# Grice-Lab/HmmUFOtu

Measured on AMD Instinct MI355X. Metric: reads placed/sec (whole node), gg_97_otus GTR+dGamma 250bp; HBM GB/s %peak, higher is better.
Workload: dtype f64; 1 GPU; gg_97_otus-scale synthetic DB (198643 nodes x 7682 CS columns, K=1400), GTR+dGamma(4), SE 250 bp amplicon reads, batch 8192 reads/step/GPU, 6 batches in flight, seeds in the reference's std::sort order (k_seed_refsort); seed_order=reference, message_window_cols=7682, parallelism=read-sharded x1

## Files before the change

hmmufotu_amd/csrc/hu_engine.hip:

```cpp
#include <algorithm>
#include <cmath>
#include <cstdio>
#include <cstring>
#include <limits>
#include <map>
#include <atomic>
#include <thread>
#include <memory>
#include <mutex>
#include <chrono>
#include <fstream>
#include <sstream>
#include <new>
#include <stdexcept>
#include <fcntl.h>
#include <unistd.h>
#include "hu_common.h"
#include "hu_kern_sep.h"
#include "hu_kern_align.h"
#include "hu_kern_tree.h"
#include "hu_kern_blk.h"
#include "hu_kern_refsort.h"
#include "hu_kern_rank.h"
#include "hu_kern_anneal.h"
// ... 1667 lines not shown
	bool fixedRoot = false;
	bool placesGiven = false;
	bool pair16 = false;
	int scanWidth = 0;
	int pairsKind = 0;
	int seedCap = HU_MAX_SEEDS;
	hipStream_t stream = nullptr;
	hipEvent_t ev[2 * HU_T_COUNT];
	bool evSet[HU_T_COUNT] = {false};
	float ms[HU_T_COUNT];
	double wall[4] = {0, 0, 0, 0};
	DBuf<char> dBases, dTraces, dRows;
	DBuf<HuReadDesc> dDescs;
	DBuf<double> dScratch;
	DBuf<uint8_t> dDec;
	DBuf<HuVitOut> dVit;
	DBuf<HuAlnDev> dAlns;
	DBuf<int8_t> dCodes;
	DBuf<int32_t> dStart, dEnd, dSeedCnt, dSeedId, dGiven, dPermCnt;
	DBuf<uint16_t> dPerm;
	DBuf<uint32_t> dRp, dPairs, dSeedDN, dParDN, dBmin, dRSpan, dTileSpan;
	DBuf<int32_t> dTileQ, dSlotRead, dReadSlot;
	DBuf<uint32_t> dRq, dTileW;
	DBuf<unsigned long long> dRefScratch;
	DBuf<int32_t> dHv, dZeroPar; DBuf<unsigned long long> dPairsC; int refHvCount = 0; double refHvHeight = NAN;
	DBuf<int32_t> dBail, dNanCnt, dNanId; DBuf<uint32_t> dNanDN;
	int nRefBail = 0;
	DBuf<uint32_t> dRefPiv; DBuf<unsigned long long> dRefL0; bool refFused = false;
	int refHostAll = 0;
	DBuf<int32_t> dIns, dTileIns, dRetry;
	DBuf<uint32_t> dSortK, dSortV;
	DBuf<uint32_t> dCsCnt;
	DBuf<HuEstOut> dEst;
	DBuf<HuCand> dCands;
	DBuf<HuPlaceOut> dPlaceOut;
	DBuf<int32_t> dCandCnt, dCandOff, dMeta;
	DBuf<uint8_t> dFiltSlot;
	DBuf<HuPlaceRec> dPlaces;
	DBuf<hu_place_rec> dBest;
	size_t nc = 0;
	int maxGapSites = 0, maxBaseSites = 0;
	bool hostCands = false;
	DBuf<double> dRootLL;
	PinnedVec<double> hRootLL;
	std::vector<HuReadDesc> hDescs;
	std::vector<char> hBases;
	PinnedVec<HuVitOut> hVit;
	int64_t cellsTotal = 0, cornerTotal = 0;
	int rMain = 0;
	int maxAll = 1, maxMain = 1;
	std::vector<int32_t> wideReads;
	std::vector<uint32_t> hWideOrd, hWideCand; DBuf<uint32_t> dWideOrd, dWideCand;
	PinnedVec<int32_t> hCandOffAll;
	DBuf<double> dRedoScr; DBuf<HuReadDesc> dRedoDesc; DBuf<HuVitOut> dRedoVit;
	PinnedVec<HuAlnDev> hAlns;
	DBuf<int32_t> dAnRow, dAnThr, dAnTileQ; DBuf<int2> dAnReg; DBuf<uint32_t> dAnMasks; DBuf<unsigned long long> dAnHits;
	PinnedVec<int32_t> hStart, hEnd, hSeedCnt, hSeedId;
	PinnedVec<uint32_t> hSeedDN;
	PinnedVec<HuCand> hCands;
	std::vector<int64_t> candOffs;
	std::vector<HostPlace> places;
	PinnedVec<hu_place_rec> best;
	PinnedVec<int32_t> hMeta, hBail;
	PinnedVec<char> hRows;
	DBuf<uint32_t> dSumBits; DBuf<unsigned char> dSumCls; DBuf<int4> dSumOut; PinnedVec<int4> hSumOut; bool sumReady = false;
	std::vector<char> tsvBuf; std::vector<size_t> tsvOff, tsvLen; size_t tsvSize = 0;
// ... 955 lines not shown
	const int kth = tmp[W];
	static const int bounds[] = {512, 768, 1024, 1536, 2048, 3072};
	int bound = 0;
	for(int x : bounds) if(kth <= x) { bound = x; break; }
	if(!bound || bound >= b->maxAll) return;
	b->rMain = bound; b->maxMain = 1;
	for(int r = 0; r < b->n; ++r) { if(R[r] > bound) b->wideReads.push_back(r); else b->maxMain = std::max(b->maxMain, R[r]); }
	if(b->knob.trace) fprintf(stderr, "[hu] width split: %zu of %d reads beyond %d columns (widest %d) take a launch of their own\n", b->wideReads.size(), b->n, bound, b->maxAll);
}
static HuDbDev width_pass_dev(const hu_batch* b, int pass, const uint32_t* wideList) {
	HuDbDev dev = b->db->dev;
	if(b->rMain) { dev.rLo = pass ? b->rMain : -1; dev.rHi = pass ? 0x7fffffff : b->rMain; dev.wideList = pass ? wideList : nullptr; }
	return dev;
}

extern "C" int hu_estimate_batch(hu_batch* b, const hu_opts* o) try {
	if(!b || !o) return HU_ERR_ARG;
	if(b->state < ST_SEEDED) { hu_set_error("hu_estimate_batch: no seeds"); return HU_ERR_STATE; }
	HIPCHK(hipSetDevice(b->db->device));
	const size_t n = (size_t) b->n;
	int rc;
	if((rc = b->dEst.ensure(n * HU_MAX_SEEDS)) != HU_OK) return rc;
	(void) hipGetLastError();
	if(n) {
		Timer t(b, HU_T_ESTIMATE);
		plan_width_split(b);
		const bool stream = b->knob.streaming_sep != 0;
		if(b->rMain) {
			b->hWideOrd.clear();
			for(int r : b->wideReads) for(int sd = 0; sd < HU_MAX_SEEDS; ++sd) b->hWideOrd.push_back((uint32_t) r * HU_MAX_SEEDS + sd);
			if((rc = b->dWideOrd.ensure(b->hWideOrd.size())) != HU_OK) return rc;
			HIPCHK(hipMemcpyAsync(b->dWideOrd.p, b->hWideOrd.data(), b->hWideOrd.size() * 4, hipMemcpyHostToDevice, b->stream));
		}
		for(int pass = 0; pass < (b->rMain ? 2 : 1); ++pass) {
			const int maxR = pass ? b->maxAll : b->maxMain;
			const HuDbDev dev = width_pass_dev(b, pass, b->dWideOrd.p);
			#define EST_ARGS dev, b->db->mdl, b->dCodes.p, b->dStart.p, b->dEnd.p, b->dParDN.p, b->dSeedCnt.p, b->dSeedId.p, b->dSeedDN.p, o->weighted, b->dEst.p
			const unsigned eg = pass ? (unsigned) b->hWideOrd.size() : (unsigned) b->n * HU_MAX_SEEDS;
			const uint32_t* order = nullptr;
			if(pass) order = b->dWideOrd.p;
			else if(!b->knob.est_unsorted) {
				if((rc = b->dSortK.ensure((size_t) eg * 2)) != HU_OK || (rc = b->dSortV.ensure((size_t) eg * 2)) != HU_OK) return rc;
				k_seed_sortkeys<<<(eg + 255) / 256, 256, 0, b->stream>>>(b->n, b->dSeedCnt.p, b->dSeedId.p, b->dSortK.p, b->dSortV.p);
				if((rc = order_by_key(b, b->dSortK.p, b->dSortV.p, (size_t) eg, (uint32_t) b->db->dev.nNodes, b->dSortV.p + eg, false)) != HU_OK) return rc;
				order = b->dSortV.p + eg;
			}
			const int spt = (maxR + 255) / 256;
			const int xm = b->knob.xcd_map;
			const unsigned egl = pass ? eg : order ? std::min<unsigned>(eg, (unsigned) b->n * (unsigned) b->seedCap) : eg;
			const int var = b->knob.est_var;
			auto said = [&](const char* k) { if(b->knob.trace) fprintf(stderr, "[hu] estimate: max region %d, %s\n", maxR, k); };
			if(stream || spt > 12) { said("k_estimate"); k_estimate<<<eg, 64, 0, b->stream>>>(EST_ARGS); }
			else if(var == 2) {
				if(spt <= 2) { said("k_estimate_blk<2,256>"); k_estimate_blk<2, 256><<<eg, 256, 0, b->stream>>>(EST_ARGS); }
				else if(spt <= 4) { said("k_estimate_blk<4,256>"); k_estimate_blk<4, 256><<<eg, 256, 0, b->stream>>>(EST_ARGS); }
				else if(spt <= 6) { said("k_estimate_blk<6,256>"); k_estimate_blk<6, 256><<<eg, 256, 0, b->stream>>>(EST_ARGS); }
				else if(spt <= 8) { said("k_estimate_blk<8,256>"); k_estimate_blk<8, 256><<<eg, 256, 0, b->stream>>>(EST_ARGS); }
				else { said("k_estimate_blk<12,256>"); k_estimate_blk<12, 256><<<eg, 256, 0, b->stream>>>(EST_ARGS); }
			}
			else if(var == 98 && spt > 4 && spt <= 6) {
				said("k_estimate_prod<6,4,4,true>");
				DBuf<long long> ddb;
				if((rc = ddb.ensure((size_t) egl * 4)) != HU_OK) return rc;
				HIPCHK(hipMemsetAsync(ddb.p, 0, (size_t) egl * 4 * sizeof(long long), b->stream));
				k_estimate_prod<6, 4, 4, true><<<egl, 256, 0, b->stream>>>(EST_ARGS, order, xm, ddb.p);
				std::vector<long long> hd((size_t) egl * 4);
				HIPCHK(hipMemcpyAsync(hd.data(), ddb.p, hd.size() * sizeof(long long), hipMemcpyDeviceToHost, b->stream));
				HIPCHK(hu_wait(b->stream));
				double acc[4] = {0}; size_t ran = 0;
				for(size_t c = 0; c < (size_t) egl; ++c) if(hd[c * 4 + 3]) { ++ran; for(int i = 0; i < 4; ++i) acc[i] += (double) hd[c * 4 + i]; }
				if(ran) fprintf(stderr, "[est dbg] per slot (s_memtime ticks, %zu slots): prologue %.0f load %.0f rest %.0f total %.0f\n", ran, acc[0] / ran, acc[1] / ran, acc[2] / ran, acc[3] / ran);
			}
			else if(var == 1 && spt <= 6) { said("k_estimate_prod<12,2>"); k_estimate_prod<12, 2><<<egl, 128, 0, b->stream>>>(EST_ARGS, order, xm); }
			else if(var == 3 && spt <= 6) { said("k_estimate_prod<6,4,1>"); k_estimate_prod<6, 4, 1><<<egl, 256, 0, b->stream>>>(EST_ARGS, order, xm); }
			else if(spt <= 2) { said("k_estimate_prod<2,4>"); k_estimate_prod<2, 4><<<egl, 256, 0, b->stream>>>(EST_ARGS, order, xm); }
			else if(spt <= 4) { said("k_estimate_prod<4,4>"); k_estimate_prod<4, 4><<<egl, 256, 0, b->stream>>>(EST_ARGS, order, xm); }
			else if(spt <= 6) { said("k_estimate_prod<6,4,4>"); k_estimate_prod<6, 4, 4><<<egl, 256, (size_t)(b->knob.est_lds_pad > 0 && b->knob.est_lds_pad <= 60 ? b->knob.est_lds_pad : 0) * 1024, b->stream>>>(EST_ARGS, order, xm); }
			else if(spt <= 8) { said("k_estimate_prod<8,4>"); k_estimate_prod<8, 4><<<egl, 256, 0, b->stream>>>(EST_ARGS, order, xm); }
			else if(var == 4) { said("k_estimate_prod<12,4>"); k_estimate_prod<12, 4><<<egl, 256, 0, b->stream>>>(EST_ARGS, order, xm); }
			else { said("k_estimate_prod<6,8,2>"); k_estimate_prod<6, 8, 2><<<egl, 512, 0, b->stream>>>(EST_ARGS, order, xm); }
			#undef EST_ARGS
		}
	}
	HIPCHK(hipGetLastError());
	if(n) {
		if((rc = b->dPermCnt.ensure(n * 2)) != HU_OK) return rc;
		k_site_count<<<b->n, 64, 0, b->stream>>>(b->db->dev, b->n, b->dCodes.p, b->dStart.p, b->dEnd.p, b->dPermCnt.p);
		HIPCHK(hipGetLastError());
	}
	b->state = ST_ESTIMATED;
	return HU_OK;
} catch(...) { return hu_catch_all("hu_estimate_batch"); }


static int sync_host_cands(hu_batch* b) {
	if(b->hostCands) return HU_OK;
	const size_t n = (size_t) b->n;
	std::vector<int32_t> off(n + 1, 0);
	b->places.resize(b->nc);
	HIPCHK(hipSetDevice(b->db->device));
	if(n) HIPCHK(hipMemcpyAsync(off.data(), b->dCandOff.p, (n + 1) * 4, hipMemcpyDeviceToHost, b->stream));
	if(b->nc) HIPCHK(hipMemcpyAsync(b->places.data(), b->dPlaces.p, b->nc * sizeof(HuPlaceRec), hipMemcpyDeviceToHost, b->stream));
	HIPCHK(hu_wait(b->stream));
	b->candOffs.assign(off.begin(), off.end());
	b->hostCands = true;
	return HU_OK;
}
static int scan_cands(hu_batch* b, bool withPerm) {
	int rc;
	if((rc = b->dCandOff.ensure((size_t) b->n + 1)) != HU_OK || (rc = b->dMeta.ensure(4)) != HU_OK) return rc;
	k_cand_scan<<<1, 1024, 0, b->stream>>>(b->n, b->dCandCnt.p, b->dCandOff.p, withPerm ? b->dPermCnt.p : nullptr, b->dStart.p, b->dEnd.p, b->dMeta.p, b->rMain);
	HIPCHK(hipGetLastError());
	b->hMeta.assign(4, 0);
	int32_t* meta = b->hMeta.data();
// ... 708 lines not shown
		HIPCHK(hu_wait(b->stream));
	}
	for(size_t r = 0; r < n; ++r) {
		if(n_seeds) n_seeds[r] = cnt[r];
		for(int s = 0; s < HU_MAX_SEEDS && s < stride; ++s) {
			const bool ok = s < cnt[r];
			const size_t k = r * HU_MAX_SEEDS + s, w = r * (size_t) stride + s;
			if(ids) ids[w] = ok ? id[k] : -1;
			if(d) d[w] = ok ? (int32_t)(dn[k] >> 16) : 0;
			if(N) N[w] = ok ? (int32_t)(dn[k] & 0xffffu) : 0;
		}
	}
	return HU_OK;
} catch(...) { return hu_catch_all("hu_batch_get_seeds_strided"); }
extern "C" int hu_batch_get_estimates_strided(hu_batch* b, double* ratio, double* wnr, double* loglik, int stride) try {
	if(!b || stride < 1) return HU_ERR_ARG;
	if(b->state < ST_ESTIMATED) { hu_set_error("no estimates yet"); return HU_ERR_STATE; }
	HIPCHK(hipSetDevice(b->db->device));
	const size_t n = (size_t) b->n;
	std::vector<HuEstOut> e(n * HU_MAX_SEEDS); std::vector<int32_t> cnt(n);
	if(n) {
		HIPCHK(hipMemcpyAsync(e.data(), b->dEst.p, e.size() * sizeof(HuEstOut), hipMemcpyDeviceToHost, b->stream));
		HIPCHK(hipMemcpyAsync(cnt.data(), b->dSeedCnt.p, n * 4, hipMemcpyDeviceToHost, b->stream));
		HIPCHK(hu_wait(b->stream));
	}
	for(size_t r = 0; r < n; ++r) for(int s = 0; s < HU_MAX_SEEDS && s < stride; ++s) {
		const size_t k = r * HU_MAX_SEEDS + s, w = r * (size_t) stride + s; const bool ok = s < cnt[r];
		if(ratio) ratio[w] = ok ? e[k].ratio : NAN;
		if(wnr) wnr[w] = ok ? e[k].wnr : NAN;
		if(loglik) loglik[w] = ok ? e[k].loglik : NAN;
	}
	return HU_OK;
} catch(...) { return hu_catch_all("hu_batch_get_estimates_strided"); }
extern "C" int hu_batch_get_candidates(hu_batch* b, int64_t* offs, int32_t* c_node, double* ratio, double* wnr, double* est_loglik, int32_t* iters) try {
	if(!b) return HU_ERR_ARG;
	if(b->state < ST_FILTERED) { hu_set_error("no candidates yet"); return HU_ERR_STATE; }
	{ const int rc = sync_host_cands(b); if(rc != HU_OK) return rc; }
	if(offs) memcpy(offs, b->candOffs.data(), b->candOffs.size() * 8);
	for(size_t c = 0; c < b->places.size(); ++c) {
		const HostPlace& p = b->places[c];
		if(c_node) c_node[c] = p.cNode; if(ratio) ratio[c] = p.ratio; if(wnr) wnr[c] = p.wnr;
		if(est_loglik) est_loglik[c] = p.estLoglik; if(iters) iters[c] = p.iters;
	}
	return HU_OK;
} catch(...) { return hu_catch_all("hu_batch_get_candidates"); }
static hu_place_rec to_rec(const HostPlace& p, int32_t nCand) {
	hu_place_rec r;
	r.c_node = p.cNode; r.p_node = p.pNode; r.a_node = p.aNode; r.n_cand = nCand;
	r.wuv = p.wuv; r.ratio = p.ratio; r.wnr = p.wnr; r.loglik = p.loglik; r.height = p.height;
	r.q_place = p.qPlace; r.q_taxon = p.qTaxon; r.anno_dist = p.annoDist(); r.est_loglik = p.estLoglik; r.root_loglik = p.rootLoglik;
	return r;
}
extern "C" int hu_batch_get_candidate_places(hu_batch* b, hu_place_rec* recs) try {
	if(!b || !recs) return HU_ERR_ARG;
	if(b->state < ST_FINISHED) { hu_set_error("batch is not finished"); return HU_ERR_STATE; }
	{ const int rc = sync_host_cands(b); if(rc != HU_OK) return rc; }
	for(size_t r = 0; r + 1 < b->candOffs.size(); ++r)
		for(int64_t c = b->candOffs[r]; c < b->candOffs[r + 1]; ++c) recs[c] = to_rec(b->places[c], (int32_t)(b->candOffs[r + 1] - b->candOffs[r]));
	return HU_OK;
} catch(...) { return hu_catch_all("hu_batch_get_candidate_places"); }
extern "C" int hu_batch_get_placements(hu_batch* b, hu_place_rec* best) try {
	if(!b || !best) return HU_ERR_ARG;
	if(b->state < ST_FINISHED) { hu_set_error("batch is not finished"); return HU_ERR_STATE; }
	memcpy(best, b->best.data(), b->best.size() * sizeof(hu_place_rec));
	return HU_OK;
} catch(...) { return hu_catch_all("hu_batch_get_placements"); }
// ... 407 lines not shown
```

hmmufotu_amd/csrc/hu_kern_blk.h:

```cpp
#pragma once
#include "hu_kern_sep.h"

#define HU_BLK_THREADS 256

__device__ inline void lds_wave_sync() { asm volatile("s_waitcnt lgkmcnt(0)" ::: "memory"); }
__device__ inline void lds_barrier() { asm volatile("s_waitcnt lgkmcnt(0)\n\ts_barrier" ::: "memory"); }

template<int NW = 4>
__device__ inline double block_sum(double v, double* red, int& phase) {
	v = wave_sum_uniform(v);
	double* r = red + (phase & 1) * NW;
	if((threadIdx.x & 63) == 0) r[threadIdx.x >> 6] = v;
	lds_barrier();
	double s = r[0];
#pragma unroll
	for(int w = 1; w < NW; ++w) s += r[w];
	phase ^= 1;
	return s;
}
template<int NW = 4>
__device__ inline long long block_sum_ll(long long v, long long* red, int& phase) {
	for(int m = 32; m > 0; m >>= 1) v += __shfl_xor(v, m);
	long long* r = red + (phase & 1) * NW;
	if((threadIdx.x & 63) == 0) r[threadIdx.x >> 6] = v;
// ... 97 lines not shown
	if(tid == 0) { HuEstOut o; o.ratio = ratio; o.wnr = wnr; o.loglik = ll; out[(size_t) read * HU_MAX_SEEDS + s] = o; }
}

template<int CTRL>
__device__ inline double dpp_mul_full(double v) {
	const int lo = __builtin_amdgcn_mov_dpp(__double2loint(v), CTRL, 0xf, 0xf, true);
	const int hi = __builtin_amdgcn_mov_dpp(__double2hiint(v), CTRL, 0xf, 0xf, true);
	return v * __hiloint2double(hi, lo);
}
__device__ inline double wave_prod(double v) {
	v = dpp_mul_full<0xB1>(v);
	v = dpp_mul_full<0x4E>(v);
	v = dpp_mul_full<0x141>(v);
	v = dpp_mul_full<0x140>(v);
	v *= __shfl_xor(v, 16);
	v *= __shfl_xor(v, 32);
	return v;
}
__device__ inline int wave_sum_i32(int v) {
	for(int m = 32; m > 0; m >>= 1) v += __shfl_xor(v, m);
	return v;
}

__device__ inline uint32_t hu_xcd_pos(uint32_t b, uint32_t nb, int xmap) {
	if(!xmap) return b;
	const uint32_t per = nb >> 3;
	return b < per * 8 ? (b & 7u) * per + (b >> 3) : b;
}

__host__ __device__ constexpr int hu_est_waves(int spt, int occ) {
	const int w = spt <= 2 ? 8 : spt <= 4 ? 5 : spt <= 6 ? 4 : spt <= 8 ? 3 : 2;
	return occ > w ? occ : w;
}
template<int SPT, int NW, int OCC = 1, bool DBG = false>
__global__ __launch_bounds__(64 * NW, hu_est_waves(SPT, OCC)) void k_estimate_prod(HuDbDev db, HuModelDev mdl, const int8_t* __restrict__ codes,
		const int32_t* __restrict__ rstart, const int32_t* __restrict__ rend, const uint32_t* __restrict__ parDN,
		const int32_t* __restrict__ seedCnt, const int32_t* __restrict__ seedId, const uint32_t* __restrict__ seedDN,
		int weighted, HuEstOut* __restrict__ out, const uint32_t* __restrict__ order, int xmap = 0, long long* __restrict__ dbg = nullptr) {
	constexpr int THREADS = 64 * NW;
	long long tk[4] = {0, 0, 0, 0}, t0 = 0, tl = 0;
	auto stamp = [&](int i) { if(DBG) { const long long t = (long long) __builtin_amdgcn_s_memtime(); tk[i] += t - tl; tl = t; } };
	if(DBG) { t0 = tl = (long long) __builtin_amdgcn_s_memtime(); }
	__shared__ double redd[2 * NW];
	__shared__ int redi[2 * NW];
	__shared__ __attribute__((aligned(16))) double Qtab[24];
	__shared__ __attribute__((aligned(16))) double pro[12];
	__shared__ __attribute__((aligned(16))) double mtab[36];
	const uint32_t slot = order ? order[hu_xcd_pos(blockIdx.x, gridDim.x, xmap)] : blockIdx.x;
	const int read = slot / HU_MAX_SEEDS, s = slot % HU_MAX_SEEDS, tid = threadIdx.x, lane = tid & 63;
	const int wave = __builtin_amdgcn_readfirstlane(tid >> 6);
	const bool builder = wave == (int)(blockIdx.x % NW);
	if(s >= seedCnt[read] || hu_skip_width(db, rend[read] - rstart[read] + 1)) return;
	const int un = seedId[(size_t) read * HU_MAX_SEEDS + s];
	double ratio = 0;
	if(builder) {
		static_assert(offsetof(HuModelDev, U) == offsetof(HuModelDev, pi) + 64 && offsetof(HuModelDev, U1) == offsetof(HuModelDev, pi) + 192, "pi, logpi, U, U1 in a row");
		const double* __restrict__ mp = reinterpret_cast<const double*>(reinterpret_cast<const char*>(&mdl) + offsetof(HuModelDev, pi));
		const int l36 = lane < 36 ? lane : 0;
		const double mc = mp[l36 < 4 ? l36 : l36 + 4];
		const uint32_t dn = seedDN[(size_t) read * HU_MAX_SEEDS + s];
		const uint32_t pv = parDN[(size_t) read * HU_MAX_SEEDS + s];
		const double cDist = (double)(dn >> 16) / (double)(dn & 0xffffu);
		const double pDist = (double)(pv >> 16) / (double)(pv & 0xffffu);
		ratio = cDist / (cDist + pDist);
		if(isnan(ratio)) ratio = 0.5;
		ratio = __hiloint2double(__builtin_amdgcn_readfirstlane(__double2hiint(ratio)), __builtin_amdgcn_readfirstlane(__double2loint(ratio)));
		const double w0 = db.blen[un];
		const double wur = w0 * ratio, wvr = w0 - wur;
		const int l6 = lane < 6 ? lane : 0, m3 = l6 % 3;
		const double e = exp((m3 == 0 ? mdl.lam[1] : m3 == 1 ? mdl.lam[2] : mdl.lam[3]) * (l6 < 3 ? wur : wvr));
		if(lane < 6) pro[lane] = e;
		if(weighted) {
			double piw[4];
			{ double mx = max4d(mdl.logpi), sm; for(int i = 0; i < 4; ++i) piw[i] = exp(mdl.logpi[i] - mx); sm = (piw[0] + piw[2]) + (piw[1] + piw[3]); for(int i = 0; i < 4; ++i) piw[i] /= sm; }
			if(lane < 4) pro[8 + lane] = sel4(piw, lane);
		}
		if(lane < 36) mtab[lane] = mc;
	}
	const int start = rstart[read], end = rend[read], n = end - start + 1;
	const int8_t* __restrict__ cd = codes + (size_t) read * db.csLen + start;
	const int64_t sOff = (int64_t) un * db.winLen + (start - db.winStart);
	const int piMax = argmax4d(mdl.logpi);
	double z[SPT][4]; unsigned long long bop = 0; int ksum = 0;
	double Eu[3], Ev[3];
	double aU[SPT][4], aV[SPT][4];
	const double* __restrict__ Ub = db.up + sOff * 4; const double* __restrict__ Vb = db.down + sOff * 4;
	const int32_t* __restrict__ upKb = db.upK + sOff; const int32_t* __restrict__ downKb = db.downK + sOff;
	auto inr = [&](int t) { return tid < n - THREADS * t; };
	stamp(0);
	{
		int kU[SPT], kV[SPT];
#pragma unroll
		for(int t = 0; t < SPT; ++t) {
			const int jj = inr(t) ? tid + THREADS * t : 0;
			kU[t] = upKb[(size_t) jj]; kV[t] = downKb[(size_t) jj];
		}
		__builtin_amdgcn_sched_barrier(0);
#pragma unroll
		for(int t = 0; t < SPT; ++t) {
			const int jj = inr(t) ? tid + THREADS * t : 0;
			load4(Ub + (size_t) jj * 4, aU[t]); load4(Vb + (size_t) jj * 4, aV[t]);
			const int b = cd[jj];
			bop |= (unsigned long long)(b >= 0 ? b : 4) << (3 * t);
		}
		__builtin_amdgcn_sched_barrier(0);
		lds_barrier();
		{
			const double e = pro[lane < 6 ? lane : 0];
			const int lo = __double2loint(e), hi = __double2hiint(e);
#pragma unroll
			for(int k = 0; k < 3; ++k) {
				Eu[k] = __hiloint2double(__builtin_amdgcn_readlane(hi, k), __builtin_amdgcn_readlane(lo, k));
				Ev[k] = __hiloint2double(__builtin_amdgcn_readlane(hi, 3 + k), __builtin_amdgcn_readlane(lo, 3 + k));
			}
		}
#pragma unroll
		for(int t = 0; t < SPT; ++t) {
			asm volatile("" : "+v"(kU[t]), "+v"(kV[t]));
			ksum += inr(t) ? kU[t] + kV[t] : 0;
		}
	}
	if(DBG) { double x = 0; for(int t = 0; t < SPT; ++t) x += aU[t][0] + aV[t][0]; if(x == 1.2345e-300 || bop == ~0ull) tk[2] = 1; }
	stamp(1);
	{
#pragma unroll
		for(int t = 0; t < SPT; ++t) {
			const double su1 = Eu[0] * aU[t][1], su2 = Eu[1] * aU[t][2], su3 = Eu[2] * aU[t][3];
			const double sv1 = Ev[0] * aV[t][1], sv2 = Ev[1] * aV[t][2], sv3 = Ev[2] * aV[t][3];
#pragma unroll
			for(int i = 0; i < 4; ++i) {
				const double cu = fmax(fma(mdl.U[i*4+3], su3, fma(mdl.U[i*4+2], su2, fma(mdl.U[i*4+1], su1, aU[t][0]))), 0.0);
				const double cv = fmax(fma(mdl.U[i*4+3], sv3, fma(mdl.U[i*4+2], sv2, fma(mdl.U[i*4+1], sv1, aV[t][0]))), 0.0);
				z[t][i] = cu * cv;
			}
		}
	}
	double wnr = 0;
	if(!weighted) {
		int nd = 0;
#pragma unroll
		for(int t = 0; t < SPT; ++t) {
			const int bi = (int)((bop >> (3 * t)) & 7u);
			const int b1 = argmax4_tied_lin(z[t]), b2 = bi < 4 ? bi : piMax;
			nd += __popcll(__ballot(inr(t) && b1 != b2));
		}
		if(lane == 0) redi[wave] = nd;
		lds_barrier();
		if(builder) {
			int tot = redi[0];
#pragma unroll
			for(int w = 1; w < NW; ++w) tot += redi[w];
			wnr = (double) tot / (double) n;
		}
	}
	else {
		const double piwGap = pro[8 + piMax];
		double dsum = 0, nsum = 0;
#pragma unroll
		for(int t = 0; t < SPT; ++t) {
			if(!inr(t)) continue;
			const int bi = (int)((bop >> (3 * t)) & 7u);
			const int b1 = argmax4_tied_lin(z[t]), b2 = bi < 4 ? bi : piMax;
			const double w1 = sel4(z[t], b1) / ((z[t][0] + z[t][2]) + (z[t][1] + z[t][3]));
			const double w2 = bi < 4 ? 1.0 : piwGap;
			if(b1 != b2) dsum += w1 * w2;
			nsum += w1 * w2;
		}
		dsum = wave_sum(dsum); nsum = wave_sum(nsum);
		if(lane == 0) { redd[wave] = dsum; redd[NW + wave] = nsum; }
		lds_barrier();
		if(builder) {
			double a = redd[0], c = redd[NW];
#pragma unroll
			for(int w = 1; w < NW; ++w) { a += redd[w]; c += redd[NW + w]; }
			wnr = a / c;
		}
	}
	double* Q = Qtab;
	if(builder) {
		if(lane < 3) Q[1 + lane] = exp((lane == 0 ? mdl.lam[1] : lane == 1 ? mdl.lam[2] : mdl.lam[3]) * wnr);
		lds_wave_sync();
		if(lane < 20) {
			const int b = lane >> 2, i = lane & 3;
			const double* mU = mtab + 4 + i * 4, * mU1 = mtab + 20 + (b & 3);
			const double pii = mtab[i];
			double c;
			if(wnr == 0) c = b < 4 ? (i == b ? 1.0 : 0.0) : pii;
			else {
				double a0, a1, a2, a3;
				if(b < 4) { a0 = mU1[0]; a1 = mU1[4]; a2 = mU1[8]; a3 = mU1[12]; }
				else {
					a0 = (mdl.U1[0] * mdl.pi[0] + mdl.U1[1] * mdl.pi[1]) + (mdl.U1[2] * mdl.pi[2] + mdl.U1[3] * mdl.pi[3]);
					a1 = (mdl.U1[4] * mdl.pi[0] + mdl.U1[5] * mdl.pi[1]) + (mdl.U1[6] * mdl.pi[2] + mdl.U1[7] * mdl.pi[3]);
					a2 = (mdl.U1[8] * mdl.pi[0] + mdl.U1[9] * mdl.pi[1]) + (mdl.U1[10] * mdl.pi[2] + mdl.U1[11] * mdl.pi[3]);
					a3 = (mdl.U1[12] * mdl.pi[0] + mdl.U1[13] * mdl.pi[1]) + (mdl.U1[14] * mdl.pi[2] + mdl.U1[15] * mdl.pi[3]);
				}
				const double Ui1 = mU[1], Ui2 = mU[2], Ui3 = mU[3];
				c = fmax(fma(Ui3, Q[3] * a3, fma(Ui2, Q[2] * a2, fma(Ui1, Q[1] * a1, a0))), 0.0);
			}
			Q[4 + b * 4 + i] = pii * c;
		}
	}
	lds_barrier();
	double mant = 1.0; int esum = ksum;
#pragma unroll
	for(int t = 0; t < SPT; ++t) {
		const double* q = Q + 4 + ((bop >> (3 * t)) & 7u) * 4;
		double x = fmax(fma(q[3], z[t][3], fma(q[2], z[t][2], fma(q[1], z[t][1], q[0] * z[t][0]))), 0.0);
		if(!inr(t)) x = 1.0;
		mant *= __builtin_amdgcn_frexp_mant(x);
		esum += x == 0.0 ? 0 : __builtin_amdgcn_frexp_exp(x);
	}
	esum += __builtin_amdgcn_frexp_exp(mant); mant = __builtin_amdgcn_frexp_mant(mant);
	mant = wave_prod(mant);
	esum = wave_sum_i32(esum);
	if(lane == 0) { redd[wave] = mant; redi[NW + wave] = esum; }
	lds_barrier();
	if(builder && lane == 0) {
		double m = redd[0]; long long e = redi[NW];
#pragma unroll
		for(int w = 1; w < NW; ++w) { m *= redd[w]; e += redi[NW + w]; }
		HuEstOut o; o.ratio = ratio; o.wnr = wnr; o.loglik = log(m) + (double) e * HU_LN2;
		out[(size_t) read * HU_MAX_SEEDS + s] = o;
	}
	if(DBG) {
		stamp(2);
		if(builder && lane == 0) { tk[3] = tl - t0; for(int i = 0; i < 4; ++i) dbg[(size_t) blockIdx.x * 4 + i] = tk[i]; }
	}
}

#define HU_RHO_SKIP 1e60
#define HU_TP 18
#define HU_EXP_MEPS 0.99999000004999983333
#define HU_EXP_PEPS 1.00001000005000016667

__device__ inline double fast_div(double a, double b) {
	double y = __builtin_amdgcn_rcp(b);
	y = fma(fma(-b, y, 1.0), y, y);
	y = fma(fma(-b, y, 1.0), y, y);
	const double q = a * y;
	return fma(fma(-b, q, a), y, q);
}

__device__ __attribute__((noinline)) double hu_exp_call(double x) { return exp(x); }
__device__ __attribute__((noinline)) double hu_log_call(double x) { return log(x); }

template<int SPT, int NW, int EMV, int RED>
__device__ inline double em_branch_blk(const double (&rho)[SPT], int nvalidWave, double q0, double maxL,
		double* red, double* redc, int& phase, int& emIters, long long* st = nullptr) {
	long long tl = st ? (long long) __builtin_amdgcn_s_memtime() : 0;
	auto stamp = [&](int i) { if(st) { const long long t = (long long) __builtin_amdgcn_s_memtime(); st[i] += t - tl; tl = t; } };
	const int lane = threadIdx.x & 63, wave = threadIdx.x >> 6;
	double p0 = 1 - q0, p = p0, q = q0, rc = 0;
	const int em0 = emIters;
	if(lane == 0) redc[(phase & 1) * NW + wave] = (double) nvalidWave;
	for(int it = 0; it < HU_MAX_ITER && p >= 0 && p <= 1; ++it) {
// ... 330 lines not shown
```

hmmufotu_amd/engine.py:

```python
from __future__ import annotations

import ctypes as C
import os
import subprocess

import numpy as np

_HERE = os.path.dirname(os.path.abspath(__file__))
LIB_PATH = os.environ.get("HU_LIB") or os.path.join(_HERE, "libhmmufotu_amd.so")
_LIB = None

HU_MAX_SEEDS = 64
T_NAMES = ["viterbi", "align_build", "seed_pdist", "seed_topk", "estimate", "place", "_6", "_7"]
MODE = {"global": 0, "local": 1, "ngcl": 2, "cgnl": 3}


class EngineError(RuntimeError):
    pass


class ProfileDesc(C.Structure):
    _fields_ = [("K", C.c_int32), ("L", C.c_int32), ("EM", C.POINTER(C.c_double)), ("EI", C.POINTER(C.c_double)),
                ("T", C.POINTER(C.c_double)), ("p2cs", C.POINTER(C.c_int32))]

# ... 2320 lines not shown
        _chk(load_library().hu_anneal_batch(self.h, _p(rows, C.c_int32), C.c_int(n), txt, C.c_double(max_dist), _p(hn, C.c_int64), _p(hl, C.c_int64)))
        return hn, hl

    def pdist(self, read: int):
        d = np.zeros(self.db.n_nodes, np.int32); N = np.zeros(self.db.n_nodes, np.int32)
        _chk(load_library().hu_batch_get_pdist(self.h, C.c_int(read), _p(d, C.c_int32), _p(N, C.c_int32)))
        return d, N

    def seeds(self):
        n = self.n
        cnt = np.zeros(n, np.int32); ids = np.zeros((n, HU_MAX_SEEDS), np.int32); d = np.zeros_like(ids); N = np.zeros_like(ids)
        _chk(load_library().hu_batch_get_seeds(self.h, _p(cnt, C.c_int32), _p(ids, C.c_int32), _p(d, C.c_int32), _p(N, C.c_int32)))
        return cnt, ids, d, N

    def seeds_strided(self, stride: int, guard: int = 0):
        n = self.n
        cnt = np.zeros(n, np.int32)
        bufs = [np.full(n * stride + guard, -777, np.int32) for _ in range(3)]
        _chk(load_library().hu_batch_get_seeds_strided(self.h, _p(cnt, C.c_int32), *[_p(b, C.c_int32) for b in bufs], C.c_int(stride)))
        return (cnt,) + tuple(bufs)

    def estimates_strided(self, stride: int, guard: int = 0):
        n = self.n
        bufs = [np.full(n * stride + guard, -777.0) for _ in range(3)]
        _chk(load_library().hu_batch_get_estimates_strided(self.h, *[_p(b, C.c_double) for b in bufs], C.c_int(stride)))
        return tuple(bufs)

    def estimates(self):
        n = self.n
        r = np.zeros((n, HU_MAX_SEEDS)); w = np.zeros_like(r); ll = np.zeros_like(r)
        _chk(load_library().hu_batch_get_estimates(self.h, _p(r, C.c_double), _p(w, C.c_double), _p(ll, C.c_double)))
        return r, w, ll

    def candidates(self):
        offs = np.zeros(self.n + 1, np.int64)
        _chk(load_library().hu_batch_get_candidates(self.h, _p(offs, C.c_int64), None, None, None, None, None))
        m = int(offs[-1])
        c = np.zeros(m, np.int32); r = np.zeros(m); w = np.zeros(m); e = np.zeros(m); it = np.zeros(m, np.int32)
        _chk(load_library().hu_batch_get_candidates(self.h, _p(offs, C.c_int64), _p(c, C.c_int32), _p(r, C.c_double), _p(w, C.c_double),
                                                    _p(e, C.c_double), _p(it, C.c_int32)))
        return dict(offs=offs, c_node=c, ratio=r, wnr=w, est_loglik=e, iters=it)

    def placements(self):
        out = np.zeros(self.n, PLACE_DTYPE)
        _chk(load_library().hu_batch_get_placements(self.h, out.ctypes.data_as(C.c_void_p)))
        return out

    def candidate_places(self):
        offs = np.zeros(self.n + 1, np.int64)
        _chk(load_library().hu_batch_get_candidates(self.h, _p(offs, C.c_int64), None, None, None, None, None))
        out = np.zeros(int(offs[-1]), PLACE_DTYPE)
        _chk(load_library().hu_batch_get_candidate_places(self.h, out.ctypes.data_as(C.c_void_p)))
        return offs, out

    def set_candidates(self, offs, recs, placed=False):
        offs = np.ascontiguousarray(offs, np.int64); recs = np.ascontiguousarray(recs, PLACE_DTYPE)
        assert len(offs) == self.n + 1 and offs[-1] == len(recs)
        _chk(load_library().hu_batch_set_candidates(self.h, _p(offs, C.c_int64), recs.ctypes.data_as(C.c_void_p), C.c_int(int(placed))))

    def get_seed_given(self, n_seeds, ids, dist_ids=None):
        n_seeds = np.ascontiguousarray(n_seeds, np.int32); ids = np.ascontiguousarray(ids, np.int32)
        assert ids.ndim == 2 and ids.shape[0] == self.n == len(n_seeds)
        di = None
        if dist_ids is not None:
            di = np.ascontiguousarray(dist_ids, np.int32); assert di.shape == ids.shape
        _chk(load_library().hu_seed_batch_given(self.h, _p(n_seeds, C.c_int32), _p(ids, C.c_int32), _p(di, C.c_int32) if di is not None else None,
# ... 58 lines not shown
```

include/hmmufotu_amd.h:

```cpp
#ifndef HMMUFOTU_AMD_H_
#define HMMUFOTU_AMD_H_

#include <stdint.h>

#ifdef __cplusplus
extern "C" {
#endif

typedef enum {
	HU_OK = 0,
	HU_ERR_ARG = -1,
	HU_ERR_DEVICE = -2,
	HU_ERR_IO = -3,
	HU_ERR_NOMEM = -4,
	HU_ERR_STATE = -5,
	HU_ERR_NUMERIC = -6
} hu_status;

enum { HU_MODE_GLOBAL = 0, HU_MODE_LOCAL = 1, HU_MODE_NGCL = 2, HU_MODE_CGNL = 3 };
enum { HU_GTR = 0, HU_TN93 = 1, HU_HKY85 = 2, HU_F81 = 3, HU_K80 = 4, HU_JC69 = 5 };
enum { HU_PRIOR_UNIFORM = 0, HU_PRIOR_HEIGHT = 1 };

enum {
	HU_READ_OK = 1,
// ... 193 lines not shown
int hu_place_batch(hu_batch* b, const hu_opts* o);
int hu_batch_set_candidates(hu_batch* b, const int64_t* offs, const hu_place_rec* recs, int placed);
int hu_finish_batch(hu_batch* b, const hu_opts* o);
int hu_assign_batch(hu_batch* b, const hu_opts* o);

typedef struct {
	int32_t num_seg;
	int32_t reserved;
	double max_chimera_error;
	double min_chimera_lod;
} hu_chimera_opts;
typedef struct {
	int32_t checked, is_chimera;
	int32_t seg5_start, seg5_end, seg3_start, seg3_end;
	int32_t n_seg5, n_seg3;
	hu_place_rec seg5, seg3;
	double alt5_loglik, alt3_loglik;
	double lod;
} hu_chimera_rec;
void hu_default_chimera_opts(const hu_opts* o, hu_chimera_opts* co);
int hu_chimera_batch(hu_batch* b, hu_batch* work, const hu_opts* o, const hu_chimera_opts* co, hu_chimera_rec* out);

int hu_batch_set_knob(hu_batch* b, const char* name, int value);

int hu_batch_sync(hu_batch* b);

int hu_batch_get_alignments(hu_batch* b, hu_align_rec* recs, char* align , char* trace, int trace_stride);
int hu_batch_get_codes(hu_batch* b, int8_t* codes , int32_t* start, int32_t* end);
int hu_batch_get_pdist(hu_batch* b, int read, int32_t* d , int32_t* N);
int hu_batch_get_seeds(hu_batch* b, int32_t* n_seeds, int32_t* ids, int32_t* d, int32_t* N);
int hu_batch_get_estimates(hu_batch* b, double* ratio, double* wnr, double* loglik);
int hu_batch_get_seeds_strided(hu_batch* b, int32_t* n_seeds, int32_t* ids, int32_t* d, int32_t* N, int stride);
int hu_batch_get_estimates_strided(hu_batch* b, double* ratio, double* wnr, double* loglik, int stride);
int hu_batch_get_candidates(hu_batch* b, int64_t* offs, int32_t* c_node, double* ratio, double* wnr, double* est_loglik, int32_t* iters);
int hu_batch_get_placements(hu_batch* b, hu_place_rec* best );
int hu_batch_get_candidate_places(hu_batch* b, hu_place_rec* recs );

int64_t hu_batch_format_tsv(hu_batch* b, const char* const* ids, const char* const* descs, const char* const* annos,
		char* buf, int64_t cap);
int64_t hu_batch_format_tsv_chimera(hu_batch* b, const char* const* ids, const char* const* descs, const char* const* annos,
		const hu_chimera_rec* chi, int chimera_info, int which, char* buf, int64_t cap);
int64_t hu_batch_format_tsv_ptr(hu_batch* b, const char* const* ids, const char* const* descs, const char* const* annos,
		const hu_chimera_rec* chi, int chimera_info, int which, const char** text);
int hu_batch_tsv_line_lengths(hu_batch* b, int64_t* lens);
const char* hu_tsv_header_chimera(void);
const char* hu_tsv_header(void);

typedef struct { int64_t win_start, win_len; } hu_window;
int hu_windows_plan(int64_t cs_len, int n_win, int64_t overlap, hu_window* out );
int hu_route_by_seeds(const hu_db* db, int n_win, const hu_window* win, int n, const int32_t* lens, const int32_t* vpaths,
		const int32_t* mate_lens, const int32_t* mate_vpaths, int32_t* window_of_read );
int hu_route_by_region(int n_win, const hu_window* win, int n, const int32_t* cs_start, const int32_t* cs_end, int32_t* window_of_read );

enum { HU_T_VITERBI = 0, HU_T_ALIGN_BUILD = 1, HU_T_SEED_PDIST = 2, HU_T_SEED_TOPK = 3,
	HU_T_ESTIMATE = 4, HU_T_PLACE = 5, HU_T_COUNT = 8 };
int hu_batch_timings(hu_batch* b, float* ms );
int hu_batch_profile(hu_batch* b, int enable);
int hu_batch_wall(hu_batch* b, double* ms4);
int hu_batch_refsort_stats(hu_batch* b, int32_t* left_to_host, int32_t* whole_batch_on_host);

int hu_anneal_batch(hu_batch* b, const int32_t* row_of_primer, int n, const char* const* as_read, double max_dist, int64_t* hit_nodes, int64_t* hit_leaves);
int64_t hu_anneal_max_mismatch(double max_dist, int32_t len);
int hu_anneal_match_table(uint8_t* out );
const char* hu_anneal_header(void);
int hu_db_num_leaves(const hu_db* db, int64_t* n_leaves);

// ... 411 lines not shown
```

Baseline: 433,800 reads/s.

## Precompute per-slot estimate records in a prepass kernel for k_estimate_prod

A new k_est_records kernel resolves the seed order, validity checks, branch ratio and the six branch exponentials for each estimate slot. It writes them as an 80-byte aligned record and computes the pi weights once. k_estimate_prod then reads one record per block into scalar registers, replacing the dependent gather chain (order, seedCnt, rstart/rend, seedId, seedDN, parDN, blen, exp) plus an LDS broadcast and barrier in its prologue. The cost is an extra small kernel launch and record traffic per pass. A host accessor for the records is also added.

```diff
diff --git a/hmmufotu_amd/csrc/hu_engine.hip b/hmmufotu_amd/csrc/hu_engine.hip
--- a/hmmufotu_amd/csrc/hu_engine.hip
+++ b/hmmufotu_amd/csrc/hu_engine.hip
@@ -1723,6 +1723,8 @@
 	DBuf<uint32_t> dSortK, dSortV;
 	DBuf<uint32_t> dCsCnt;
 	DBuf<HuEstOut> dEst;
+	DBuf<HuEstRec> dEstRec; DBuf<double> dEstPiw;
+	size_t estRecN = 0;
 	DBuf<HuCand> dCands;
 	DBuf<HuPlaceOut> dPlaceOut;
 	DBuf<int32_t> dCandCnt, dCandOff, dMeta;
@@ -2744,6 +2746,9 @@
 			if((rc = b->dWideOrd.ensure(b->hWideOrd.size())) != HU_OK) return rc;
 			HIPCHK(hipMemcpyAsync(b->dWideOrd.p, b->hWideOrd.data(), b->hWideOrd.size() * 4, hipMemcpyHostToDevice, b->stream));
 		}
+		const size_t eg0 = n * HU_MAX_SEEDS;
+		b->estRecN = 0;
+		if((rc = b->dEstRec.ensure(eg0 + (b->rMain ? b->hWideOrd.size() : 0))) != HU_OK || (rc = b->dEstPiw.ensure(4)) != HU_OK) return rc;
 		for(int pass = 0; pass < (b->rMain ? 2 : 1); ++pass) {
 			const int maxR = pass ? b->maxAll : b->maxMain;
 			const HuDbDev dev = width_pass_dev(b, pass, b->dWideOrd.p);
@@ -2761,6 +2766,13 @@
 			const int xm = b->knob.xcd_map;
 			const unsigned egl = pass ? eg : order ? std::min<unsigned>(eg, (unsigned) b->n * (unsigned) b->seedCap) : eg;
 			const int var = b->knob.est_var;
+			HuEstRec* const rec = b->dEstRec.p + (pass ? eg0 : 0);
+			if(!(stream || spt > 12) && var != 2) {
+				k_est_records<<<(eg + 255) / 256, 256, 0, b->stream>>>(dev, b->db->mdl, eg, egl, order, b->dStart.p, b->dEnd.p, b->dParDN.p, b->dSeedCnt.p, b->dSeedId.p, b->dSeedDN.p,
+						rec, o->weighted ? b->dEstPiw.p : nullptr);
+				if(!pass) b->estRecN = eg; else if(b->estRecN == eg0) b->estRecN += eg;
+			}
+			#define PROD_ARGS dev, b->db->mdl, b->dCodes.p, rec, b->dEstPiw.p, o->weighted, b->dEst.p, (order ? xm : 0)
 			auto said = [&](const char* k) { if(b->knob.trace) fprintf(stderr, "[hu] estimate: max region %d, %s\n", maxR, k); };
 			if(stream || spt > 12) { said("k_estimate"); k_estimate<<<eg, 64, 0, b->stream>>>(EST_ARGS); }
 			else if(var == 2) {
@@ -2775,7 +2787,7 @@
 				DBuf<long long> ddb;
 				if((rc = ddb.ensure((size_t) egl * 4)) != HU_OK) return rc;
 				HIPCHK(hipMemsetAsync(ddb.p, 0, (size_t) egl * 4 * sizeof(long long), b->stream));
-				k_estimate_prod<6, 4, 4, true><<<egl, 256, 0, b->stream>>>(EST_ARGS, order, xm, ddb.p);
+				k_estimate_prod<6, 4, 4, true><<<egl, 256, 0, b->stream>>>(PROD_ARGS, ddb.p);
 				std::vector<long long> hd((size_t) egl * 4);
 				HIPCHK(hipMemcpyAsync(hd.data(), ddb.p, hd.size() * sizeof(long long), hipMemcpyDeviceToHost, b->stream));
 				HIPCHK(hu_wait(b->stream));
@@ -2783,15 +2795,16 @@
 				for(size_t c = 0; c < (size_t) egl; ++c) if(hd[c * 4 + 3]) { ++ran; for(int i = 0; i < 4; ++i) acc[i] += (double) hd[c * 4 + i]; }
 				if(ran) fprintf(stderr, "[est dbg] per slot (s_memtime ticks, %zu slots): prologue %.0f load %.0f rest %.0f total %.0f\n", ran, acc[0] / ran, acc[1] / ran, acc[2] / ran, acc[3] / ran);
 			}
-			else if(var == 1 && spt <= 6) { said("k_estimate_prod<12,2>"); k_estimate_prod<12, 2><<<egl, 128, 0, b->stream>>>(EST_ARGS, order, xm); }
-			else if(var == 3 && spt <= 6) { said("k_estimate_prod<6,4,1>"); k_estimate_prod<6, 4, 1><<<egl, 256, 0, b->stream>>>(EST_ARGS, order, xm); }
-			else if(spt <= 2) { said("k_estimate_prod<2,4>"); k_estimate_prod<2, 4><<<egl, 256, 0, b->stream>>>(EST_ARGS, order, xm); }
-			else if(spt <= 4) { said("k_estimate_prod<4,4>"); k_estimate_prod<4, 4><<<egl, 256, 0, b->stream>>>(EST_ARGS, order, xm); }
-			else if(spt <= 6) { said("k_estimate_prod<6,4,4>"); k_estimate_prod<6, 4, 4><<<egl, 256, (size_t)(b->knob.est_lds_pad > 0 && b->knob.est_lds_pad <= 60 ? b->knob.est_lds_pad : 0) * 1024, b->stream>>>(EST_ARGS, order, xm); }
-			else if(spt <= 8) { said("k_estimate_prod<8,4>"); k_estimate_prod<8, 4><<<egl, 256, 0, b->stream>>>(EST_ARGS, order, xm); }
-			else if(var == 4) { said("k_estimate_prod<12,4>"); k_estimate_prod<12, 4><<<egl, 256, 0, b->stream>>>(EST_ARGS, order, xm); }
-			else { said("k_estimate_prod<6,8,2>"); k_estimate_prod<6, 8, 2><<<egl, 512, 0, b->stream>>>(EST_ARGS, order, xm); }
+			else if(var == 1 && spt <= 6) { said("k_estimate_prod<12,2>"); k_estimate_prod<12, 2><<<egl, 128, 0, b->stream>>>(PROD_ARGS); }
+			else if(var == 3 && spt <= 6) { said("k_estimate_prod<6,4,1>"); k_estimate_prod<6, 4, 1><<<egl, 256, 0, b->stream>>>(PROD_ARGS); }
+			else if(spt <= 2) { said("k_estimate_prod<2,4>"); k_estimate_prod<2, 4><<<egl, 256, 0, b->stream>>>(PROD_ARGS); }
+			else if(spt <= 4) { said("k_estimate_prod<4,4>"); k_estimate_prod<4, 4><<<egl, 256, 0, b->stream>>>(PROD_ARGS); }
+			else if(spt <= 6) { said("k_estimate_prod<6,4,4>"); k_estimate_prod<6, 4, 4><<<egl, 256, (size_t)(b->knob.est_lds_pad > 0 && b->knob.est_lds_pad <= 60 ? b->knob.est_lds_pad : 0) * 1024, b->stream>>>(PROD_ARGS); }
+			else if(spt <= 8) { said("k_estimate_prod<8,4>"); k_estimate_prod<8, 4><<<egl, 256, 0, b->stream>>>(PROD_ARGS); }
+			else if(var == 4) { said("k_estimate_prod<12,4>"); k_estimate_prod<12, 4><<<egl, 256, 0, b->stream>>>(PROD_ARGS); }
+			else { said("k_estimate_prod<6,8,2>"); k_estimate_prod<6, 8, 2><<<egl, 512, 0, b->stream>>>(PROD_ARGS); }
 			#undef EST_ARGS
+			#undef PROD_ARGS
 		}
 	}
 	HIPCHK(hipGetLastError());
@@ -3566,6 +3579,27 @@
 	}
 	return HU_OK;
 } catch(...) { return hu_catch_all("hu_batch_get_estimates_strided"); }
+extern "C" int hu_batch_get_est_records(hu_batch* b, int64_t* count, int32_t* node, int32_t* slot, int32_t* start, int32_t* n, double* ratio, double* e) try {
+	if(!b || !count) return HU_ERR_ARG;
+	if(b->state < ST_ESTIMATED) { hu_set_error("no estimates yet"); return HU_ERR_STATE; }
+	HIPCHK(hipSetDevice(b->db->device));
+	const size_t m = b->estRecN;
+	*count = (int64_t) m;
+	if(!m || !(node || slot || start || n || ratio || e)) return HU_OK;
+	std::vector<HuEstRec> r(m);
+	HIPCHK(hipMemcpyAsync(r.data(), b->dEstRec.p, m * sizeof(HuEstRec), hipMemcpyDeviceToHost, b->stream));
+	HIPCHK(hu_wait(b->stream));
+	for(size_t p = 0; p < m; ++p) {
+		const bool ok = r[p].node >= 0;
+		if(node) node[p] = ok ? r[p].node : -1;
+		if(slot) slot[p] = ok ? (int32_t) r[p].slot : -1;
+		if(start) start[p] = ok ? r[p].start : 0;
+		if(n) n[p] = ok ? r[p].n : 0;
+		if(ratio) ratio[p] = ok ? r[p].ratio : NAN;
+		if(e) for(int k = 0; k < 6; ++k) e[p * 6 + k] = ok ? r[p].e[k] : NAN;
+	}
+	return HU_OK;
+} catch(...) { return hu_catch_all("hu_batch_get_est_records"); }
 extern "C" int hu_batch_get_candidates(hu_batch* b, int64_t* offs, int32_t* c_node, double* ratio, double* wnr, double* est_loglik, int32_t* iters) try {
 	if(!b) return HU_ERR_ARG;
 	if(b->state < ST_FILTERED) { hu_set_error("no candidates yet"); return HU_ERR_STATE; }
diff --git a/hmmufotu_amd/csrc/hu_kern_blk.h b/hmmufotu_amd/csrc/hu_kern_blk.h
--- a/hmmufotu_amd/csrc/hu_kern_blk.h
+++ b/hmmufotu_amd/csrc/hu_kern_blk.h
@@ -153,11 +153,60 @@
 	const int w = spt <= 2 ? 8 : spt <= 4 ? 5 : spt <= 6 ? 4 : spt <= 8 ? 3 : 2;
 	return occ > w ? occ : w;
 }
+struct __attribute__((aligned(16))) HuEstRec {
+	int32_t node;
+	uint32_t slot;
+	int32_t start, n;
+	double ratio;
+	double e[6];
+	double pad;
+};
+static_assert(sizeof(HuEstRec) == 80, "HuEstRec: 20 words");
+
+__global__ __launch_bounds__(256) void k_est_records(HuDbDev db, HuModelDev mdl, unsigned np, unsigned nLaunch, const uint32_t* __restrict__ order,
+		const int32_t* __restrict__ rstart, const int32_t* __restrict__ rend, const uint32_t* __restrict__ parDN,
+		const int32_t* __restrict__ seedCnt, const int32_t* __restrict__ seedId, const uint32_t* __restrict__ seedDN,
+		HuEstRec* __restrict__ rec, double* __restrict__ piwOut) {
+	const unsigned p = blockIdx.x * 256u + threadIdx.x;
+	if(p == 0 && piwOut) {
+		double piw[4];
+		{ double mx = max4d(mdl.logpi), sm; for(int i = 0; i < 4; ++i) piw[i] = exp(mdl.logpi[i] - mx); sm = (piw[0] + piw[2]) + (piw[1] + piw[3]); for(int i = 0; i < 4; ++i) piw[i] /= sm; }
+		for(int i = 0; i < 4; ++i) piwOut[i] = piw[i];
+	}
+	if(p >= np) return;
+	if(p >= nLaunch) { rec[p].node = -1; return; }
+	const uint32_t slot = order ? order[p] : p;
+	const int read = slot / HU_MAX_SEEDS, s = slot % HU_MAX_SEEDS;
+	if(s >= seedCnt[read]) { rec[p].node = -1; return; }
+	const int start = rstart[read], n = rend[read] - start + 1;
+	if(hu_skip_width(db, n)) { rec[p].node = -1; return; }
+	const int un = seedId[slot];
+	const uint32_t dn = seedDN[slot];
+	const uint32_t pv = parDN[slot];
+	const double cDist = (double)(dn >> 16) / (double)(dn & 0xffffu);
+	const double pDist = (double)(pv >> 16) / (double)(pv & 0xffffu);
+	double ratio = cDist / (cDist + pDist);
+	if(isnan(ratio)) ratio = 0.5;
+	const double w0 = db.blen[un];
+	const double wur = w0 * ratio, wvr = fma(-w0, ratio, w0);
+	HuEstRec r;
+	r.node = un; r.slot = slot; r.start = start; r.n = n; r.ratio = ratio; r.pad = 0;
+#pragma unroll
+	for(int m = 0; m < 3; ++m) {
+		double xu, xv;
+		{
+#pragma clang fp contract(off)
+			xu = mdl.lam[1 + m] * wur; xv = mdl.lam[1 + m] * wvr;
+		}
+		r.e[m] = exp(xu); r.e[3 + m] = exp(xv);
+	}
+	rec[p] = r;
+}
+
 template<int SPT, int NW, int OCC = 1, bool DBG = false>
 __global__ __launch_bounds__(64 * NW, hu_est_waves(SPT, OCC)) void k_estimate_prod(HuDbDev db, HuModelDev mdl, const int8_t* __restrict__ codes,
-		const int32_t* __restrict__ rstart, const int32_t* __restrict__ rend, const uint32_t* __restrict__ parDN,
-		const int32_t* __restrict__ seedCnt, const int32_t* __restrict__ seedId, const uint32_t* __restrict__ seedDN,
-		int weighted, HuEstOut* __restrict__ out, const uint32_t* __restrict__ order, int xmap = 0, long long* __restrict__ dbg = nullptr) {
+		const HuEstRec* __restrict__ rec, const double* __restrict__ piwBuf,
+		int weighted, HuEstOut* __restrict__ out, int xmap = 0, long long* __restrict__ dbg = nullptr) {
 	constexpr int THREADS = 64 * NW;
 	long long tk[4] = {0, 0, 0, 0}, t0 = 0, tl = 0;
 	auto stamp = [&](int i) { if(DBG) { const long long t = (long long) __builtin_amdgcn_s_memtime(); tk[i] += t - tl; tl = t; } };
@@ -165,40 +214,25 @@
 	__shared__ double redd[2 * NW];
 	__shared__ int redi[2 * NW];
 	__shared__ __attribute__((aligned(16))) double Qtab[24];
-	__shared__ __attribute__((aligned(16))) double pro[12];
 	__shared__ __attribute__((aligned(16))) double mtab[36];
-	const uint32_t slot = order ? order[hu_xcd_pos(blockIdx.x, gridDim.x, xmap)] : blockIdx.x;
-	const int read = slot / HU_MAX_SEEDS, s = slot % HU_MAX_SEEDS, tid = threadIdx.x, lane = tid & 63;
+	const HuEstRec* __restrict__ rp = rec + hu_xcd_pos(blockIdx.x, gridDim.x, xmap);
+	const int4 hd = *reinterpret_cast<const int4*>(rp);
+	double ratio = rp->ratio, re0 = rp->e[0], re1 = rp->e[1], re2 = rp->e[2], re3 = rp->e[3], re4 = rp->e[4], re5 = rp->e[5];
+	asm volatile("" : "+s"(ratio), "+s"(re0), "+s"(re1), "+s"(re2), "+s"(re3), "+s"(re4), "+s"(re5));
+	const int un = hd.x;
+	if(un < 0) return;
+	const uint32_t slot = (uint32_t) hd.y;
+	const int read = slot / HU_MAX_SEEDS, tid = threadIdx.x, lane = tid & 63;
 	const int wave = __builtin_amdgcn_readfirstlane(tid >> 6);
 	const bool builder = wave == (int)(blockIdx.x % NW);
-	if(s >= seedCnt[read] || hu_skip_width(db, rend[read] - rstart[read] + 1)) return;
-	const int un = seedId[(size_t) read * HU_MAX_SEEDS + s];
-	double ratio = 0;
+	double mc = 0;
 	if(builder) {
 		static_assert(offsetof(HuModelDev, U) == offsetof(HuModelDev, pi) + 64 && offsetof(HuModelDev, U1) == offsetof(HuModelDev, pi) + 192, "pi, logpi, U, U1 in a row");
 		const double* __restrict__ mp = reinterpret_cast<const double*>(reinterpret_cast<const char*>(&mdl) + offsetof(HuModelDev, pi));
 		const int l36 = lane < 36 ? lane : 0;
-		const double mc = mp[l36 < 4 ? l36 : l36 + 4];
-		const uint32_t dn = seedDN[(size_t) read * HU_MAX_SEEDS + s];
-		const uint32_t pv = parDN[(size_t) read * HU_MAX_SEEDS + s];
-		const double cDist = (double)(dn >> 16) / (double)(dn & 0xffffu);
-		const double pDist = (double)(pv >> 16) / (double)(pv & 0xffffu);
-		ratio = cDist / (cDist + pDist);
-		if(isnan(ratio)) ratio = 0.5;
-		ratio = __hiloint2double(__builtin_amdgcn_readfirstlane(__double2hiint(ratio)), __builtin_amdgcn_readfirstlane(__double2loint(ratio)));
-		const double w0 = db.blen[un];
-		const double wur = w0 * ratio, wvr = w0 - wur;
-		const int l6 = lane < 6 ? lane : 0, m3 = l6 % 3;
-		const double e = exp((m3 == 0 ? mdl.lam[1] : m3 == 1 ? mdl.lam[2] : mdl.lam[3]) * (l6 < 3 ? wur : wvr));
-		if(lane < 6) pro[lane] = e;
-		if(weighted) {
-			double piw[4];
-			{ double mx = max4d(mdl.logpi), sm; for(int i = 0; i < 4; ++i) piw[i] = exp(mdl.logpi[i] - mx); sm = (piw[0] + piw[2]) + (piw[1] + piw[3]); for(int i = 0; i < 4; ++i) piw[i] /= sm; }
-			if(lane < 4) pro[8 + lane] = sel4(piw, lane);
-		}
-		if(lane < 36) mtab[lane] = mc;
-	}
-	const int start = rstart[read], end = rend[read], n = end - start + 1;
+		mc = mp[l36 < 4 ? l36 : l36 + 4];
+	}
+	const int start = hd.z, n = hd.w;
 	const int8_t* __restrict__ cd = codes + (size_t) read * db.csLen + start;
 	const int64_t sOff = (int64_t) un * db.winLen + (start - db.winStart);
 	const int piMax = argmax4d(mdl.logpi);
@@ -210,31 +244,25 @@
 	auto inr = [&](int t) { return tid < n - THREADS * t; };
 	stamp(0);
 	{
-		int kU[SPT], kV[SPT];
+		int kU[SPT], kV[SPT], cb[SPT];
 #pragma unroll
 		for(int t = 0; t < SPT; ++t) {
 			const int jj = inr(t) ? tid + THREADS * t : 0;
 			kU[t] = upKb[(size_t) jj]; kV[t] = downKb[(size_t) jj];
 		}
+#pragma unroll
+		for(int t = 0; t < SPT; ++t) cb[t] = cd[inr(t) ? tid + THREADS * t : 0];
 		__builtin_amdgcn_sched_barrier(0);
 #pragma unroll
 		for(int t = 0; t < SPT; ++t) {
 			const int jj = inr(t) ? tid + THREADS * t : 0;
 			load4(Ub + (size_t) jj * 4, aU[t]); load4(Vb + (size_t) jj * 4, aV[t]);
-			const int b = cd[jj];
-			bop |= (unsigned long long)(b >= 0 ? b : 4) << (3 * t);
 		}
 		__builtin_amdgcn_sched_barrier(0);
-		lds_barrier();
-		{
-			const double e = pro[lane < 6 ? lane : 0];
-			const int lo = __double2loint(e), hi = __double2hiint(e);
-#pragma unroll
-			for(int k = 0; k < 3; ++k) {
-				Eu[k] = __hiloint2double(__builtin_amdgcn_readlane(hi, k), __builtin_amdgcn_readlane(lo, k));
-				Ev[k] = __hiloint2double(__builtin_amdgcn_readlane(hi, 3 + k), __builtin_amdgcn_readlane(lo, 3 + k));
-			}
-		}
+#pragma unroll
+		for(int t = 0; t < SPT; ++t) bop |= (unsigned long long)(cb[t] >= 0 ? cb[t] : 4) << (3 * t);
+		if(builder && lane < 36) mtab[lane] = mc;
+		Eu[0] = re0; Eu[1] = re1; Eu[2] = re2; Ev[0] = re3; Ev[1] = re4; Ev[2] = re5;
 #pragma unroll
 		for(int t = 0; t < SPT; ++t) {
 			asm volatile("" : "+v"(kU[t]), "+v"(kV[t]));
@@ -275,7 +303,7 @@
 		}
 	}
 	else {
-		const double piwGap = pro[8 + piMax];
+		const double piwGap = piwBuf[piMax];
 		double dsum = 0, nsum = 0;
 #pragma unroll
 		for(int t = 0; t < SPT; ++t) {
@@ -342,7 +370,7 @@
 #pragma unroll
 		for(int w = 1; w < NW; ++w) { m *= redd[w]; e += redi[NW + w]; }
 		HuEstOut o; o.ratio = ratio; o.wnr = wnr; o.loglik = log(m) + (double) e * HU_LN2;
-		out[(size_t) read * HU_MAX_SEEDS + s] = o;
+		out[slot] = o;
 	}
 	if(DBG) {
 		stamp(2);
diff --git a/hmmufotu_amd/engine.py b/hmmufotu_amd/engine.py
--- a/hmmufotu_amd/engine.py
+++ b/hmmufotu_amd/engine.py
@@ -2376,6 +2376,17 @@
         _chk(load_library().hu_batch_get_estimates(self.h, _p(r, C.c_double), _p(w, C.c_double), _p(ll, C.c_double)))
         return r, w, ll
 
+    def est_records(self):
+        cnt = C.c_int64(0)
+        _chk(load_library().hu_batch_get_est_records(self.h, C.byref(cnt), None, None, None, None, None, None))
+        m = int(cnt.value)
+        node = np.zeros(m, np.int32); slot = np.zeros(m, np.int32); start = np.zeros(m, np.int32); n = np.zeros(m, np.int32)
+        ratio = np.zeros(m); e = np.zeros((m, 6))
+        if m:
+            _chk(load_library().hu_batch_get_est_records(self.h, C.byref(cnt), _p(node, C.c_int32), _p(slot, C.c_int32), _p(start, C.c_int32),
+                                                         _p(n, C.c_int32), _p(ratio, C.c_double), _p(e, C.c_double)))
+        return dict(node=node, slot=slot, start=start, n=n, ratio=ratio, e=e)
+
     def candidates(self):
         offs = np.zeros(self.n + 1, np.int64)
         _chk(load_library().hu_batch_get_candidates(self.h, _p(offs, C.c_int64), None, None, None, None, None))
diff --git a/include/hmmufotu_amd.h b/include/hmmufotu_amd.h
--- a/include/hmmufotu_amd.h
+++ b/include/hmmufotu_amd.h
@@ -249,6 +249,7 @@
 int hu_batch_get_estimates(hu_batch* b, double* ratio, double* wnr, double* loglik);
 int hu_batch_get_seeds_strided(hu_batch* b, int32_t* n_seeds, int32_t* ids, int32_t* d, int32_t* N, int stride);
 int hu_batch_get_estimates_strided(hu_batch* b, double* ratio, double* wnr, double* loglik, int stride);
+int hu_batch_get_est_records(hu_batch* b, int64_t* count, int32_t* node, int32_t* slot, int32_t* start, int32_t* n, double* ratio, double* e);
 int hu_batch_get_candidates(hu_batch* b, int64_t* offs, int32_t* c_node, double* ratio, double* wnr, double* est_loglik, int32_t* iters);
 int hu_batch_get_placements(hu_batch* b, hu_place_rec* best );
 int hu_batch_get_candidate_places(hu_batch* b, hu_place_rec* recs );
```

Result: no change. 437,300 reads/s (median of 6 runs) (+0.8%).
